# opteroncx/MoePhoto

Hardware: AMD Instinct MI355X
Metric: megapixels/sec (input), 1080p 4x SR (Net4x a4), 256-px tiles with overlap (higher is better)
Workload: dtype fp16; 1 GPU; BASELINE configs[1]: 1 frame(s) 1920x1080 RGB -> 7680x4320, model a4 (Net4x, synthetic weights in zoo format), crop 256 pad 5 align 8 -> 40 tiles/frame, fp16 I/O, fp16 MFMA operands + fp32 accumulate; tiles_per_frame=40, parallelism=single GPU, precision=mixed, exact_blocks=1, input=natural-image-like synthetic frame (tests/golden_defs.natural_image)

## Files before the change

### moephoto_amd/build.py

```python
import hashlib
import os
import subprocess
import sys

HERE = os.path.dirname(os.path.abspath(__file__))
CSRC = os.path.join(HERE, 'csrc')
SOURCES = ['conv_mfma.hip', 'conv3x3_sp.hip', 'conv3x3_rw.hip', 'conv3x3_ps4.hip', 'conv3x3_ps9.hip', 'arsb32c.hip', 'conv64_x3.hip', 'conv64_q8.hip', 'conv64_sq.hip', 'arsb_sq.hip', 'conv64_s.hip', 'conv1x1.hip', 'conv1x1_f2.hip', 'misc_kernels.hip', 'blend.hip', 'sym.hip',
           'errors.cpp', 'options.cpp', 'weights.cpp', 'forward.cpp', 'forward_arsb.cpp', 'forward_sedn.cpp', 'forward_lite.cpp', 'calibrate.cpp', 'plan_run.cpp', 'planner.cpp']
HEADERS = ['common.h', 'engine.h', 'net.h', 'rowtile.h', os.path.join('..', '..', 'include', 'moephoto_amd.h')]
LIB = os.path.join(HERE, 'libmoephoto_amd.so')
ARCH = 'gfx950'
EXTRA_FLAGS = {'blend.hip': ['-ffp-contract=off'],
               'sym.hip': ['-ffp-contract=off'],
               'arsb32c.hip': ['-fno-slp-vectorize', '-fno-honor-nans', '-mllvm', '-amdgpu-mfma-vgpr-form=1'], 'conv64_x3.hip': ['-fno-slp-vectorize'], 'conv64_q8.hip': ['-fno-slp-vectorize', '-fno-honor-nans', '-mllvm', '-amdgpu-mfma-vgpr-form=1'], 'conv64_sq.hip': ['-fno-slp-vectorize', '-fno-honor-nans', '-mllvm', '-amdgpu-mfma-vgpr-form=1'], 'arsb_sq.hip': ['-fno-slp-vectorize', '-fno-honor-nans', '-mllvm', '-amdgpu-mfma-vgpr-form=1'], 'conv64_s.hip': ['-fno-slp-vectorize', '-fno-honor-nans', '-mllvm', '-amdgpu-mfma-vgpr-form=1'], 'conv1x1.hip': ['-fno-slp-vectorize', '-mllvm', '-amdgpu-mfma-vgpr-form=1'], 'conv1x1_f2.hip': ['-fno-slp-vectorize', '-mllvm', '-amdgpu-mfma-vgpr-form=1'], 'conv3x3_sp.hip': ['-fno-honor-nans'], 'conv3x3_rw.hip': ['-fno-honor-nans', '-fno-slp-vectorize'],
               'conv3x3_ps4.hip': ['-fno-honor-nans', '-fno-slp-vectorize', '-mllvm', '-amdgpu-mfma-vgpr-form=1'],
               'conv3x3_ps9.hip': ['-fno-honor-nans', '-fno-slp-vectorize', '-mllvm', '-amdgpu-mfma-vgpr-form=1']}


def hipcc():
    for c in (os.environ.get('HIPCC'), '/opt/rocm/bin/hipcc', 'hipcc'):
        if c and (os.path.isabs(c) and os.path.exists(c) or not os.path.isabs(c)):
            return c
    return 'hipcc'


def source_digest():
    import hashlib
    h = hashlib.sha256()
    for f in sorted(SOURCES + HEADERS[:-1]) + HEADERS[-1:]:
        h.update(f.encode())
        h.update(open(os.path.join(CSRC, f), 'rb').read())
    return h.hexdigest()


def _compile_cmd(src, extra=()):
    obj = os.path.join(HERE, '_obj', os.path.splitext(src)[0] + '.o')
    cmd = [hipcc(), '--offload-arch=' + ARCH, '-O3', '-std=c++17', '-fPIC', '-x', 'hip', '-c', os.path.join(CSRC, src), '-o', obj]
    cmd += ['-cuid=moe_' + os.path.splitext(src)[0]]
    cmd += EXTRA_FLAGS.get(src, []) + list(extra)
    rel = [c.replace(CSRC, '<csrc>').replace(HERE, '<pkg>') for c in cmd[1:]]
    return cmd, hashlib.sha256('\0'.join(rel).encode()).hexdigest()


def stale():
    if not os.path.exists(LIB):
        return True
    t = os.path.getmtime(LIB)
    for src in SOURCES:
        tag = os.path.join(HERE, '_obj', os.path.splitext(src)[0] + '.o.cmd')
        if not os.path.exists(tag) or open(tag).read().strip() != _compile_cmd(src)[1]:
            return True
    return os.environ.get('MOE_HIPCC_FLAGS') is not None or any(os.path.getmtime(os.path.join(CSRC, f)) > t for f in SOURCES + HEADERS)


def build_lib(force=False, verbose=False):
    if not force and not stale():
        return LIB
    objs = []
    os.makedirs(os.path.join(HERE, '_obj'), exist_ok=True)
    keep = {os.path.splitext(src)[0] + e for src in SOURCES for e in ('.o', '.o.cmd')}
    for old in os.listdir(os.path.join(HERE, '_obj')):
        if old not in keep:
# ... 55 lines not shown
```

### moephoto_amd/csrc/conv3x3_ps4.hip

```cpp
#include "common.h"
#include "rowtile.h"
#include "../../include/moephoto_amd.h"
#include <algorithm>
#include <type_traits>

#ifndef PS4_FILL
#define PS4_FILL 5
#endif
#ifndef PS4_ZSKIP
#define PS4_ZSKIP 1
#endif
#ifndef PS4_ABL
#define PS4_ABL 0
#endif

namespace {

constexpr int RB = 4;
constexpr int PW = kTileW + 2;
constexpr int ROWB = PW * 128;
constexpr int BLKB = RB * ROWB;
constexpr int NPIECE = BLKB / 1024;
constexpr int TREC = 36 * 128 + 64;
constexpr int TEXP = 36 * 128;
constexpr int TROWS = 16;
constexpr int OFF_T = 2 * BLKB;
constexpr int OFF_BIAS = OFF_T + TROWS * TREC;
constexpr int OFF_TW = OFF_BIAS + 1024;
constexpr int OFF_DUMP = OFF_TW + 8 * 1024;
constexpr int LDS_BYTES = OFF_DUMP + 1024;

typedef unsigned u4_t __attribute__((ext_vector_type(4)));
typedef unsigned u2_t __attribute__((ext_vector_type(2)));
typedef float float2_t __attribute__((ext_vector_type(2)));
typedef const __attribute__((address_space(3))) half8_t* lds_h8_t;

enum OpKind : int { OP_NONE = 0, OP_P, OP_WL, OP_TM, OP_TW, OP_BI, OP_DMA, OP_FA, OP_FR, OP_FS, OP_AR, OP_AS, OP_ST };
struct Op { int kind, a, b, c; };
struct OpList {
    int n = 0;
    Op op[64] = {};
    constexpr void push(int kind, int a = 0, int b = 0, int c = 0) { op[n] = Op{kind, a, b, c}; ++n; }
    constexpr void append(const OpList& o) { for (int i = 0; i < o.n; ++i) { op[n] = o.op[i]; ++n; } }
};
constexpr OpList row_ops(int epi)
{
    OpList r;
    if (epi == 0) {
        for (int s = 0; s < 4; ++s) {
            r.push(OP_P, s >> 1, 4 * (s & 1), 2); r.push(OP_P, s >> 1, 4 * (s & 1) + 2, 2);
            r.push(OP_ST, s >> 1, s & 1);
        }
        return r;
    }
    const bool split = epi == 2;
    int nl = 0;
    auto wl = [&](int frag) { r.push(OP_WL, frag, nl & 1); ++nl; };
    int nt = 0;
    wl(0);
    wl(split ? 4 : 1);
    for (int s = 0; s < 4; ++s) {
        if (split) for (int k = 0; k < 4; ++k) r.push(OP_P, s >> 1, 4 * (s & 1) + k, 1);
        else for (int k = 0; k < 4; k += 2) r.push(OP_P, s >> 1, 4 * (s & 1) + k, 2);
        r.push(OP_TM, nt & 1, 0, nt == 0); ++nt;
        if (split) {
            if (s < 3) wl(s + 1);
            r.push(OP_TM, nt & 1, 1, 0); ++nt;
            if (s < 3) wl(4 + s + 1);
        } else if (s + 2 < 4) wl(s + 2);
    }
    for (int k = 0; k < 5; ++k) r.push(OP_TW, k);
// ... 91 lines not shown
    };
    auto piece_off = [&](int ya, int xa, bool live) {
        const bool ok = ((unsigned)(ya + (int)d_r) < (unsigned)H) & ((unsigned)(xa + (int)d_cc) < (unsigned)W) & live;
        return ok ? d_off : kOOR;
    };

    unsigned fa[3];
#pragma unroll
    for (int dx = 0; dx < 3; ++dx) {
        const int cc = j + dx, z = (cc >> 1) & 7;
        fa[dx] = lds0 + (unsigned)(cc * 128 + ((z ^ hh) << 4));
        asm volatile("" : "+v"(fa[dx]));
    }
    unsigned wa[5];
#pragma unroll
    for (int k = 0; k < 5; ++k) {
        const int t = k < 4 ? 4 * hh + k : 8;
        const int dy = t / 3, dx = t - 3 * dy;
        int col = j;
        if (pj == 1 && dx == 0) col = j + 1;
        if (pj == 0 && dx == 2) col = j - 1;
        unsigned o = (unsigned)((w4 * 9 + t) * 128 + col * 4);
        if (col == kTileW) o = (unsigned)(TEXP + ((0 * 2 + pi) * 3 + dy) * 4);
        if (col < 0) o = (unsigned)(TEXP + ((1 * 2 + pi) * 3 + dy) * 4);
        if (k == 4 && hh == 1) o = (unsigned)(TEXP + 48 + w4 * 4);
        wa[k] = lds0 + (unsigned)OFF_T + o;
        asm volatile("" : "+v"(wa[k]));
    }
    const int f_i = (lane >> 4) & 1, f_xp = lane & 15;
    const int a_side = (lane >> 1) & 1, a_i = lane & 1;
    unsigned slope2;
    {
        const half2_t s2 = {(half_t)a.slope, (half_t)a.slope};
        slope2 = __builtin_bit_cast(unsigned, s2);
    }
    const float16_t zero16 = {0.f, 0.f, 0.f, 0.f, 0.f, 0.f, 0.f, 0.f, 0.f, 0.f, 0.f, 0.f, 0.f, 0.f, 0.f, 0.f};

    float16_t acc[4][2];
    half8_t fr[3];
    half8_t twr[2];
    unsigned hX[4], lX[4];
    float16_t Gt = zero16;

    asm volatile("s_waitcnt lgkmcnt(0)" ::: "memory");
    __builtin_amdgcn_s_barrier();

    while (item < item_end) {
        const int s0 = item % nyb;
        const int t_ = item / nyb;
        const int pxi = t_ % px, b = t_ / px;
        const int s1 = min(nyb, s0 + (item_end - item));
        item += s1 - s0;
        const int x0 = pxi * kTileW;
        const int nblk = s1 - s0 + 3;
        const int kfirst = (PS4_ZSKIP && s0 == 0) ? 1 : 0;
        const int kz = (PS4_ZSKIP && s1 == nyb) ? nblk - 2 : nblk - 1;
        const bool okx = x0 + j < W;
        const int ylo = RB * s0, yhi = RB * s1;

        asm volatile("s_waitcnt lgkmcnt(0)" ::: "memory");
        __builtin_amdgcn_s_barrier();
        asm volatile("" ::: "memory");
        {
            const int ya = RB * (s0 - 1 + kfirst), xa = x0 - 1;
            const unsigned org = (unsigned)((b * H + ya + RB) * W + xa + 1) * 128u;
#pragma unroll
            for (int m = 0; m < 5; ++m) {
                piece_addr(m);
                const bool mine = m < 4 || w4 == 0;
                char* dst = smem + (m < 4 ? (w4 + 4 * m) * 1024 : (mine ? 16 * 1024 : OFF_DUMP));
                __builtin_amdgcn_raw_ptr_buffer_load_lds(rin, (__attribute__((address_space(3))) void*)dst, 16, piece_off(ya, xa, mine), org, 0, 0);
#if PS4_ABL & 128
                if (m < 4) __builtin_amdgcn_raw_ptr_buffer_load_lds(rin, (__attribute__((address_space(3))) void*)(dst + BLKB), 16, piece_off(ya + 4 * RB, xa, mine), org + (unsigned)(4 * RB * W) * 128u, 0, 0);
#endif
            }
#pragma unroll
            for (int s = 0; s < 4; ++s)
#pragma unroll
                for (int cg = 0; cg < 2; ++cg) acc[s][cg] = *(const __attribute__((address_space(3))) float16_t*)(bias_ad + cg * 128);
            asm volatile("s_waitcnt vmcnt(0) lgkmcnt(0)" ::: "memory");
            __builtin_amdgcn_s_barrier();
            asm volatile("" ::: "memory");
            fr[0] = *(lds_h8_t)(fa[0]);
            fr[1] = *(lds_h8_t)(fa[0] ^ 32u);
        }

        auto block = [&](int k, auto BUF_, auto KIND_) __attribute__((always_inline)) {
            constexpr int BUF = decltype(BUF_)::value;
            constexpr bool LAST = decltype(KIND_)::value == 2;
            constexpr bool ZERO = decltype(KIND_)::value == 1;
            const int Rk = RB * (s0 - 1 + k);
            const bool live = k + 1 < kz;
            const int yan = Rk + RB, xan = x0 - 1;
            const unsigned orgn = (unsigned)__builtin_amdgcn_readfirstlane((int)((unsigned)((b * H + yan + RB) * W + xan + 1) * 128u));
            const int yf = Rk - 7 + w4;
            const bool f_ok = (yf >= ylo) & (yf < yhi);
            unsigned fb[3];
            float2_t fs[2] = {{0.f, 0.f}, {0.f, 0.f}};
            float2_t fv[2];
            float av[3];

            auto step = [&](auto E_) __attribute__((always_inline)) {
                constexpr int e = decltype(E_)::value;
                const int orow = Rk + e - 2;
                const unsigned trow = (unsigned)__builtin_amdgcn_readfirstlane((int)((unsigned)((orow + 64) & 15) * (unsigned)TREC));
                const bool rowok = (unsigned)orow < (unsigned)H;
                constexpr int SL = (e + 2) & 3;

                auto op_p = [&](auto CG_, auto K0_, auto N_) __attribute__((always_inline)) {
                    constexpr int cg = decltype(CG_)::value, k0 = decltype(K0_)::value, n = decltype(N_)::value;
#pragma unroll
                    for (int k = k0; k < k0 + n; ++k) {
                        const float s0v = acc[SL][cg][2 * k], s1v = acc[SL][cg][2 * k + 1];
                        unsigned hv, lv = 0;
                        if (SPLIT) {
                            const float t0 = __builtin_fmaxf(s0v, s0v * a.slope), t1 = __builtin_fmaxf(s1v, s1v * a.slope);
                            split2(t0, t1, -2048.f, hv, lv);
                        } else {
                            const half2_t pr = {(half_t)s0v, (half_t)s1v};
                            const half2_t t = pr * __builtin_bit_cast(half2_t, slope2);
                            hv = __builtin_bit_cast(unsigned, __builtin_elementwise_max(pr, t));
                        }
                        hX[k & 3] = hv; lX[k & 3] = lv;
                    }
                };
                auto op_st = [&](auto CG_, auto G_) __attribute__((always_inline)) {
                    constexpr int cg = decltype(CG_)::value, gq = decltype(G_)::value;
                    const bool rok = (orow >= ylo) & (orow < yhi);
                    const unsigned vo = okx ? (unsigned)(2 * j) * 128u + (unsigned)hh * 16u : kOOR;
                    const unsigned so = rok ? ((unsigned)((b * 2 * H + 2 * orow + pi) * 2 * W + 2 * x0 + pj) * 128u + (unsigned)(64 * cg + 32 * gq)) : kOOR;
                    const u4_t d = {hX[0], hX[1], hX[2], hX[3]};
                    __builtin_amdgcn_raw_buffer_store_b128(d, rpl, vo, so, 0);
                };
                auto op_wl = [&](auto F_, auto S_) __attribute__((always_inline)) {
                    constexpr int fg = decltype(F_)::value, st = decltype(S_)::value;
                    twr[st] = *(lds_h8_t)(tw_ad + (unsigned)(fg * 1024));
                };
                auto op_tm = [&](auto S_, auto LO_, auto FIRST_) __attribute__((always_inline)) {
                    constexpr int st = decltype(S_)::value, lo = decltype(LO_)::value, first = decltype(FIRST_)::value;
                    const half8_t bv = lo ? __builtin_bit_cast(half8_t, u4_t{lX[0], lX[1], lX[2], lX[3]}) : __builtin_bit_cast(half8_t, u4_t{hX[0], hX[1], hX[2], hX[3]});
                    Gt = __builtin_amdgcn_mfma_f32_32x32x16_f16(twr[st], bv, first ? zero16 : Gt, 0, 0, 0);
                };
                auto op_tw = [&](auto K_) __attribute__((always_inline)) {
                    constexpr int k = decltype(K_)::value;
                    float t = __builtin_fmaf(Gt[8 + k], 0.00048828125f, Gt[k]);
                    const bool ok = MASK ? (rowok & okx) : rowok;
                    t = ok ? t : 0.f;
                    const unsigned ad = wa[k] + trow;
                    asm volatile("ds_write_b32 %0, %1" ::"v"(ad), "v"(t) : "memory");
                };
                auto op_bi = [&](auto CG_) __attribute__((always_inline)) {
                    constexpr int cg = decltype(CG_)::value;
#pragma unroll
                    for (int q = 0; q < 4; ++q) {
                        const float4_t t = *(const __attribute__((address_space(3))) float4_t*)(bias_ad + (unsigned)(cg * 128 + q * 16));
                        acc[SL][cg][4 * q] = t[0]; acc[SL][cg][4 * q + 1] = t[1]; acc[SL][cg][4 * q + 2] = t[2]; acc[SL][cg][4 * q + 3] = t[3];
// ... 12 lines not shown
#pragma unroll
                    for (int dy = 0; dy < 3; ++dy) {
                        const int isrc = f_i == 0 ? (dy == 1 ? 0 : 1) : (dy == 1 ? 1 : 0);
                        const int dd = f_i == 0 ? (dy == 0 ? -1 : 0) : (dy == 2 ? 1 : 0);
                        fb[dy] = lds0 + (unsigned)OFF_T + (unsigned)((yf + dd + 64) & 15) * (unsigned)TREC + (unsigned)((2 * isrc * 9 + dy * 3) * 128 + f_xp * 8);
                    }
                };
                auto op_fr = [&](auto DY_, auto DX_) __attribute__((always_inline)) {
                    constexpr int dy = decltype(DY_)::value, dx = decltype(DX_)::value;
                    constexpr int j0 = dx == 1 ? 0 : 1, j1 = dx == 1 ? 1 : 0;
                    if constexpr (dx > 0 || dy > 0) { fs[0] = fs[0] + fv[0]; fs[1] = fs[1] + fv[1]; }
                    fv[0] = *(const __attribute__((address_space(3))) float2_t*)(fb[dy] + (unsigned)((j0 * 9 + dx) * 128));
                    fv[1] = *(const __attribute__((address_space(3))) float2_t*)(fb[dy] + (unsigned)((j1 * 9 + dx) * 128));
                };
                auto op_fs = [&]() __attribute__((always_inline)) {
                    fs[0] = fs[0] + fv[0]; fs[1] = fs[1] + fv[1];
                    const float4_t o4 = {fs[0][0], fs[1][0], fs[0][1], fs[1][1]};
                    const bool ok = f_ok & (lane < 32) & (x0 + 2 * f_xp < W);
                    const unsigned vo = ok ? (unsigned)(f_i * 2 * W + 4 * f_xp) * 4u : kOOR;
                    const unsigned so = (unsigned)(((b * 2 * H + 2 * yf) * 2 * W) + 2 * x0) * 4u;
                    __builtin_amdgcn_raw_buffer_store_b128(__builtin_bit_cast(u4_t, o4), rpl, vo, f_ok ? so : 0u, 0);
                };
                auto op_ar = [&]() __attribute__((always_inline)) {
#pragma unroll
                    for (int dy = 0; dy < 3; ++dy) {
                        const int isrc = a_i == 0 ? (dy == 1 ? 0 : 1) : (dy == 1 ? 1 : 0);
                        const int dd = a_i == 0 ? (dy == 0 ? -1 : 0) : (dy == 2 ? 1 : 0);
                        const unsigned ad = lds0 + (unsigned)OFF_T + (unsigned)((yf + dd + 64) & 15) * (unsigned)TREC + (unsigned)(TEXP + ((a_side * 2 + isrc) * 3 + dy) * 4);
                        av[dy] = *(const __attribute__((address_space(3))) float*)ad;
                    }
                };
                auto op_as = [&]() __attribute__((always_inline)) {
                    const float v = (av[0] + av[1]) + av[2];
                    const bool ok = f_ok & (lane >= 32) & (lane < 36);
                    const unsigned vo = ok ? (unsigned)(((a_side * a.B) * px) * 2 * H + a_i) * 4u : kOOR;
                    const unsigned so = (unsigned)((b * px + pxi) * 2 * H + 2 * yf) * 4u;
                    __builtin_amdgcn_raw_buffer_store_b32(__builtin_bit_cast(unsigned, v), rap, vo, f_ok ? so : 0u, 0);
                };

                if constexpr (LAST) {
                    if constexpr (e == 0 && !(PS4_ABL & 2)) {
                        op_fa();
                        op_fr(std::integral_constant<int, 0>{}, std::integral_constant<int, 0>{}); op_fr(std::integral_constant<int, 0>{}, std::integral_constant<int, 1>{}); op_fr(std::integral_constant<int, 0>{}, std::integral_constant<int, 2>{});
                        op_fr(std::integral_constant<int, 1>{}, std::integral_constant<int, 0>{}); op_fr(std::integral_constant<int, 1>{}, std::integral_constant<int, 1>{}); op_fr(std::integral_constant<int, 1>{}, std::integral_constant<int, 2>{});
                        op_fr(std::integral_constant<int, 2>{}, std::integral_constant<int, 0>{}); op_fr(std::integral_constant<int, 2>{}, std::integral_constant<int, 1>{}); op_fr(std::integral_constant<int, 2>{}, std::integral_constant<int, 2>{});
                        op_fs();
                        op_ar(); op_as();
                    }
                    return;
                }
                auto chunk = [&](auto F_) __attribute__((always_inline)) {
                    constexpr int f = decltype(F_)::value;
                    constexpr int dx = f >> 2, ks = f & 3;
                    if (e == 3 && f == 10 && !(PS4_ABL & 16)) {
                        asm volatile("s_waitcnt vmcnt(0) lgkmcnt(0)" ::: "memory");
                        __builtin_amdgcn_s_barrier();
                        asm volatile("" ::: "memory");
                    }
                    constexpr OpList LM = row_ops(EPI);
                    constexpr OpList LX = extra_ops(e, TAIL);
                    auto half = [&](auto HC_) __attribute__((always_inline)) {
                        constexpr int hc = decltype(HC_)::value;
                        if constexpr (!ZERO) {
#pragma unroll
                            for (int u = 3 * hc; u < 3 * hc + 3; ++u) {
                                const int dy = u >> 1, cg = u & 1;
                                const int sl = (e + 1 - dy + 4) & 3;
                                acc[sl][cg] = __builtin_amdgcn_mfma_f32_32x32x16_f16(wf[cg][(dy * 3 + dx) * 4 + ks], fr[f % 3], acc[sl][cg], 0, 0, 0);
                            }
                        }
                        if constexpr (hc == 0 && !ZERO) {
                            constexpr int f2 = (f + 2) % 12;
                            constexpr int rowsel = f + 2 < 12 ? BUF * RB + e : (e < 3 ? BUF * RB + e + 1 : (BUF ^ 1) * RB);
                            if (!(PS4_ABL & 8)) fr[(f + 2) % 3] = *(lds_h8_t)((fa[f2 >> 2] ^ (unsigned)((f2 & 3) * 32)) + (unsigned)(rowsel * ROWB));
                        }
                        constexpr int h = 2 * f + hc;
                        constexpr int MH = TAIL ? 20 : 10;
                        constexpr int m_lo = h < MH ? h * LM.n / MH : LM.n, m_hi = h < MH ? (h + 1) * LM.n / MH : LM.n;
                        constexpr int x_lo = TAIL ? h * LX.n / 24 : (h < 12 ? 0 : (h - 12) * LX.n / 12), x_hi = TAIL ? (h + 1) * LX.n / 24 : (h < 12 ? 0 : (h - 11) * LX.n / 12);
                        auto runm = [&](auto I_) __attribute__((always_inline)) {
                            constexpr int I = decltype(I_)::value;
                            if constexpr (I >= m_lo && I < m_hi && !(PS4_ABL & 1)) {
                                constexpr Op o = LM.op[I];
                                if constexpr (o.kind == OP_P) op_p(std::integral_constant<int, o.a>{}, std::integral_constant<int, o.b>{}, std::integral_constant<int, o.c>{});
                                if constexpr (o.kind == OP_WL) op_wl(std::integral_constant<int, o.a>{}, std::integral_constant<int, o.b>{});
                                if constexpr (o.kind == OP_TM && !(PS4_ABL & 32)) op_tm(std::integral_constant<int, o.a>{}, std::integral_constant<int, o.b>{}, std::integral_constant<int, o.c>{});
                                if constexpr (o.kind == OP_TW) op_tw(std::integral_constant<int, o.a>{});
                                if constexpr (o.kind == OP_ST) op_st(std::integral_constant<int, o.a>{}, std::integral_constant<int, o.b>{});
                            }
                        };
                        auto runx = [&](auto I_) __attribute__((always_inline)) {
                            constexpr int I = decltype(I_)::value;
                            if constexpr (I >= x_lo && I < x_hi) {
                                constexpr Op o = LX.op[I];
                                if constexpr (o.kind != OP_DMA && (PS4_ABL & 2)) return;
                                if constexpr (o.kind == OP_DMA && (PS4_ABL & 64)) return;
                                if constexpr (o.kind == OP_DMA) op_dma(std::integral_constant<int, o.a>{}, std::integral_constant<int, o.b>{});
                                if constexpr (o.kind == OP_FA) op_fa();
                                if constexpr (o.kind == OP_FR) op_fr(std::integral_constant<int, o.a>{}, std::integral_constant<int, o.b>{});
                                if constexpr (o.kind == OP_FS) op_fs();
                                if constexpr (o.kind == OP_AR) op_ar();
                                if constexpr (o.kind == OP_AS) op_as();
                            }
                        };
#define PS4_M(I) runm(std::integral_constant<int, I>{});
                        PS4_M(0) PS4_M(1) PS4_M(2) PS4_M(3) PS4_M(4) PS4_M(5) PS4_M(6) PS4_M(7) PS4_M(8) PS4_M(9) PS4_M(10) PS4_M(11) PS4_M(12) PS4_M(13) PS4_M(14) PS4_M(15)
                        PS4_M(16) PS4_M(17) PS4_M(18) PS4_M(19) PS4_M(20) PS4_M(21) PS4_M(22) PS4_M(23) PS4_M(24) PS4_M(25) PS4_M(26) PS4_M(27) PS4_M(28) PS4_M(29) PS4_M(30) PS4_M(31)
                        PS4_M(32) PS4_M(33) PS4_M(34) PS4_M(35) PS4_M(36) PS4_M(37) PS4_M(38) PS4_M(39) PS4_M(40) PS4_M(41) PS4_M(42) PS4_M(43) PS4_M(44) PS4_M(45) PS4_M(46) PS4_M(47)
#undef PS4_M
#define PS4_X(I) runx(std::integral_constant<int, I>{});
                        PS4_X(0) PS4_X(1) PS4_X(2) PS4_X(3) PS4_X(4) PS4_X(5) PS4_X(6) PS4_X(7) PS4_X(8) PS4_X(9) PS4_X(10) PS4_X(11) PS4_X(12) PS4_X(13) PS4_X(14) PS4_X(15)
#undef PS4_X
                        if (f == 10 && hc == 1 && !(PS4_ABL & 4)) op_bi(std::integral_constant<int, 0>{});
                        if (f == 11 && hc == 1 && !(PS4_ABL & 4)) op_bi(std::integral_constant<int, 1>{});
                    };
                    half(std::integral_constant<int, 0>{});
                    half(std::integral_constant<int, 1>{});
#ifndef PS4_NOPIN
#pragma unroll
                    for (int hc = 0; hc < (ZERO ? 0 : 2); ++hc) {
                        const int h = 2 * f + hc;
                        const int MH = TAIL ? 20 : 10;
                        const int m_lo = h < MH ? h * LM.n / MH : LM.n, m_hi = h < MH ? (h + 1) * LM.n / MH : LM.n;
                        const int ntm = (PS4_ABL & 33) ? 0 : count_kind(LM, m_lo, m_hi, OP_TM);
#pragma unroll
                        for (int i_ = 0; i_ < 3; ++i_) {
                            __builtin_amdgcn_sched_group_barrier(0x008, 1, 0);
                            if (i_ == 0 && hc == 0) __builtin_amdgcn_sched_group_barrier(0x100, 1, 0);
                            __builtin_amdgcn_sched_group_barrier(0x006, PS4_FILL, 0);
                        }
#pragma unroll
                        for (int i_ = 0; i_ < 2; ++i_)
                            if (TAIL && i_ < ntm) { __builtin_amdgcn_sched_group_barrier(0x008, 1, 0); __builtin_amdgcn_sched_group_barrier(0x006, PS4_FILL, 0); }
                    }
#endif
                    __builtin_amdgcn_sched_barrier(0);
                };
#if PS4_ABL
                if constexpr (!LAST) asm volatile("" ::"v"(acc[SL][0]), "v"(acc[SL][1]), "v"(Gt));
#endif
#define PS4_CHUNK(F) chunk(std::integral_constant<int, F>{});
                PS4_CHUNK(0) PS4_CHUNK(1) PS4_CHUNK(2) PS4_CHUNK(3) PS4_CHUNK(4) PS4_CHUNK(5) PS4_CHUNK(6) PS4_CHUNK(7) PS4_CHUNK(8) PS4_CHUNK(9) PS4_CHUNK(10) PS4_CHUNK(11)
#undef PS4_CHUNK
            };
            step(std::integral_constant<int, 0>{});
            step(std::integral_constant<int, 1>{});
            step(std::integral_constant<int, 2>{});
            step(std::integral_constant<int, 3>{});
        };

        typedef std::integral_constant<int, 0> Run;
        typedef std::integral_constant<int, 1> Zero;
        typedef std::integral_constant<int, 2> Last;
        int k = kfirst;
        for (; k + 1 < kz; k += 2) {
            block(k, std::integral_constant<int, 0>{}, Run{});
            block(k + 1, std::integral_constant<int, 1>{}, Run{});
        }
        if (k < kz) { block(k, std::integral_constant<int, 0>{}, Run{}); ++k; }
        if (k < nblk - 1) { block(k, std::integral_constant<int, 0>{}, Zero{}); ++k; }
        if (TAIL) block(k, std::integral_constant<int, 0>{}, Last{});
    }
#endif
}

template <bool VEC>
__global__ __launch_bounds__(256) void tailadd_kernel(TailAddArgs a)
{
    const int nq = a.W >> 3;
    const long long idx = (long long)blockIdx.x * 256 + threadIdx.x;
    if (idx >= (long long)a.B * a.H * nq) return;
    const int xq = (int)(idx % nq);
    const int Y = (int)((idx / nq) % a.H), b = (int)(idx / ((long long)nq * a.H));
    const int X0 = xq * 8;
    const long long po = ((long long)b * a.H + Y) * a.W + X0;
    float v[8];
    {
        const float4 r0 = *(const float4*)(a.p0 + po), r1 = *(const float4*)(a.p0 + po + 4);
        v[0] = r0.x; v[1] = r0.y; v[2] = r0.z; v[3] = r0.w; v[4] = r1.x; v[5] = r1.y; v[6] = r1.z; v[7] = r1.w;
        if (a.p1) {
            const float4 u0 = *(const float4*)(a.p1 + po), u1 = *(const float4*)(a.p1 + po + 4);
            v[0] += u0.x; v[1] += u0.y; v[2] += u0.z; v[3] += u0.w; v[4] += u1.x; v[5] += u1.y; v[6] += u1.z; v[7] += u1.w;
        }
    }
    const int c = X0 >> 6, in = X0 & 63;
    const long long as = (long long)a.B * a.px * a.H;
    if (in == 0 && c >= 1) {
        const long long o = ((long long)b * a.px + (c - 1)) * a.H + Y;
        float t = a.a0[o];
        if (a.a1) t += a.a1[o];
        v[0] += t;
    }
    if (in == 56 && c + 1 < a.px) {
        const long long o = as + ((long long)b * a.px + (c + 1)) * a.H + Y;
        float t = a.a0[o];
        if (a.a1) t += a.a1[o];
        v[7] += t;
    }
    const long long yo = (a.y_off ? a.y_off[b] : (long long)b * a.H * a.W) + (long long)Y * a.W + X0;
    if (a.y_dtype == MOE_F16) {
        if (VEC) {
            half8_t h;
#pragma unroll
            for (int k = 0; k < 8; ++k) h[k] = (half_t)v[k];
            *(half8_t*)((half_t*)a.y + yo) = h;
        } else {
#pragma unroll
            for (int k = 0; k < 8; ++k) ((half_t*)a.y)[yo + k] = (half_t)v[k];
        }
    } else {
        float* yp = (float*)a.y + yo;
        if (VEC) {
            *(float4*)yp = make_float4(v[0], v[1], v[2], v[3]);
// ... 70 lines not shown
```

### moephoto_amd/csrc/forward.cpp

```cpp
#include "net.h"

using namespace moe;

namespace moe {

const char* kernel_name(ConvKernel k)
{
    static const char* const names[] = {"no kernel", "conv_direct", "conv1x1", "conv_mfma", "conv3x3_sp", "conv3x3_rw", "conv3x3_ps4 (store form)", "conv3x3_sp (hi + lo residual)",
                                        "conv_mfma (three products)", "conv64_x3", "conv64_q8", "conv64_sq", "conv3x3_sp (three launches)", "conv_mfma (fp32 side buffer)"};
    return names[(int)k];
}

static bool fast_layer(const moe_net& n, const ConvLayer& L) { return L.taps == 9 && L.nseg == 1 && !L.per_plane && n.opt.conv_impl == 2; }

ConvForm Fwd::form(const ConvLayer& L, int H, int W) const
{
    ConvForm c;
    c.B = B; c.H = H; c.W = W; c.in_cs = 64 * L.nseg; c.out_cs = L.r > 1 ? 64 : 64 * L.nchunks; c.r = L.r; c.nchunks = L.nchunks;
    c.py = (H + kTileH - 1) / kTileH;
    const long long items = (long long)B * ((W + kTileW - 1) / kTileW) * c.py;
    const int per_xcd = groups / 8;
    int G = per_xcd >= L.nchunks ? 8 * (per_xcd / L.nchunks) : groups / L.nchunks;
    if (G < 1) G = 1;
    if (G > items) G = (int)items;
    c.G = G;
    c.slope = L.slope; c.scale = L.scale; c.dbg = n.opt.dbg;
    return c;
}

ConvRoute Fwd::route(const std::string& key, const Act& in, const Act& out, const Act* res, int H, int W, const ConvExtra& e) const
{
    ConvRoute r;
    auto take = [&r](ConvKernel k) { r.kernel = k; return r; };
    auto refuse = [&r]() { r.kernel = ConvKernel::none; r.done.ok = false; return r; };
    const ConvLayer& L = n.convs[n.conv_index.at(key)];
    const bool x3 = this->x3 || e.exact;
    const bool res_lo = res && res->has_lo;
    const bool any8 = in.lo8 || out.lo8 || (res && res->lo8);
    if (any8 && !(x3 && use_q8() && q8_capable(L) && !direct)) return refuse();
    if (e.fuse_tail1) r.done.tail1_parts = 2;
    ConvForm& c = r.form;
    c = form(L, H, W);
    if (direct) return take(ConvKernel::direct);
    const int px = (W + kTileW - 1) / kTileW;
    c.res = res != nullptr; c.tail1 = e.fuse_tail1;
    c.tail = e.fuse_tail; c.tail_form = e.fuse_tail ? tail_form : 0; c.tail_split = (e.fuse_tail && mixed && tail_split_for(key)) ? 1 : 0;
    if (e.pool && !x3 && L.r == 1 && L.nchunks == 1 && !res && pooled_groups_ok((long long)c.py, (long long)B * c.py, groups)) {
        c.pool = true; c.pool_slabs = e.pool_slabs;
        c.G = pooled_groups((long long)c.py, (long long)B * c.py, groups);
    }
    const bool fast = fast_layer(n, L);
    if (e.fuse_tail && !(fast && !x3)) return refuse();
    if (n.opt.conv1x1 && L.taps == 1 && L.nseg == 1 && !L.per_plane && !res && L.scale == 1.f && !e.fuse_tail && n.opt.conv_impl == 2 && (!x3 || (in.has_lo && L.has_x3)) &&
        conv1x1_applicable(Conv1x1Form{B, H, W, L.r, L.nchunks, c.out_cs, L.slope, x3, e.fuse_tail1, x3 && out.has_lo}, groups)) {
        if (e.fuse_tail1) r.done.tail1_parts = 1;
        return take(ConvKernel::conv1x1);
    }
    const bool traced = !x3 && (c.dbg & 64) && fast && key == n.opt.trace_key;
    if (!x3 && !traced && res_lo && out.has_lo) {
        c.acc_mode = 3; c.side16 = true; c.out_lo = true;
        r.done.ok = fast && conv3x3_sp_applicable(c);
        return take(ConvKernel::sp_res_lo);
    }
    if (!x3) {
        if (c.tail && c.tail_form == 1) { r.done.ok = conv3x3_rw_applicable(c); return take(ConvKernel::rw); }
        if (fast && n.opt.up_impl == 1 && !c.tail && !c.pool && c.r == 2 && c.nchunks == 4 && c.in_cs == 64 && !c.res && c.scale == 1.f && !c.dbg && L.has_bias &&
            (long long)B * px * (H / 4) >= 32ll * groups && ps4_store_applicable(B, H, W, L.slope))
            return take(ConvKernel::ps4_store);
        if (fast && n.opt.sp_impl && !c.tail && conv3x3_rw_applicable(c)) { r.done.pooled = c.pool; return take(ConvKernel::rw); }
        if (fast && conv3x3_sp_applicable(c)) return take(ConvKernel::sp);
        if (c.tail) return refuse();
        return take(ConvKernel::mfma);
    }
    if (L.has_x3 && !fast) return take(ConvKernel::mfma_x3);
    if (n.opt.x3_fuse && fast && L.w_arsb_lo && in.has_lo && out.has_lo && (!res || res_lo) && !e.fuse_tail && !L.has_bias) {
        ConvX3Form q;
        q.B = B; q.H = H; q.W = W; q.slope = L.slope; q.res = res != nullptr; q.res_lo = res_lo;
        const long long P = (long long)px * c.py;
        if (e.pool && !res && (L.slope == 1.f || e.pool_act) && pooled_groups_ok(P, (long long)B * P, groups)) { q.pool = true; q.pool_slabs = e.pool_slabs; }
        if (e.gate && res && !use_q8()) q.gate = true;
        r.x3 = q;
        if (use_q8() && L.wq_hi8 && !q.pool && (!res || res->lo8 == in.lo8)) {
            r.x3.in8 = in.lo8; r.x3.out8 = out.lo8;
            if (n.opt.q8_impl == 1 && conv64_sq_applicable(r.x3, groups)) return take(ConvKernel::sq);
            if (conv64_q8_applicable(r.x3)) return take(ConvKernel::q8);
            r.x3 = q;
        }
        if (any8) return refuse();
        if (conv64_x3_applicable(q, groups)) { r.done.pooled = q.pool; r.done.gated = q.gate; return take(ConvKernel::x3); }
    }
    if (fast && L.nchunks <= 16) {
        ConvForm q1 = c; q1.res = res_lo; q1.slope = 1.f; q1.scale = 1.f; q1.tail = false;
        ConvForm q2 = q1; q2.res = true;
        ConvForm q3 = c; q3.acc_mode = 3; q3.side16 = true; q3.out_lo = out.has_lo;
        if (conv3x3_sp_applicable(q1) && conv3x3_sp_applicable(q2) && conv3x3_sp_applicable(q3)) return take(ConvKernel::sp_three);
    }
    if (!acc32_elems) return refuse();
    return take(ConvKernel::acc32);
}

int Fwd::launch(const ConvRoute& r, const std::string& key, const Act& in, const Act& out, const Act* res, const ConvExtra& e)
{
    const ConvLayer& L = n.convs[n.conv_index.at(key)];
    const ConvForm& c = r.form;
    const int H = c.H, W = c.W;
    if (r.kernel == ConvKernel::direct) {
        DirectConvArgs d{};
        d.in = in.hi; d.out = out.hi; d.res = res ? res->hi : nullptr;
        d.w = blob<float>(L.w_plain);
        d.bias = L.has_bias ? blob<float>(L.bias_plain) : nullptr;
        d.w_batch_stride = 0;
        d.B = B; d.H = H; d.W = W; d.in_cs = c.in_cs; d.out_cs = c.out_cs; d.cin = L.cin; d.cout = L.cout; d.k = L.k; d.r = L.r;
        d.slope = L.slope; d.scale = L.scale;
        if (L.per_plane) { d.w = (const float*)e.plane_w; d.w_batch_stride = (long long)L.cout * L.cin; }
        launch_conv_direct(d, s);
        return MOE_OK;
    }
    ConvArgs a{};
    a.in = in.hi; a.out = out.hi; a.res = res ? res->hi : nullptr;
    a.wpk = L.per_plane ? e.plane_w : blob<half_t>(L.w_hi);
    a.bias = L.has_bias ? blob<float>(L.bias) : small<float>("zero_bias");
    a.zero = small<half_t>("zero");
    a.bias_img = blob<float>(L.bias_img);
    a.trash = small<half_t>("trash");
    a.w_batch_stride = L.per_plane ? (long long)L.nchunks * L.nfrag() * 512 : 0;
    a.B = B; a.H = H; a.W = W; a.in_cs = c.in_cs; a.out_cs = c.out_cs; a.r = c.r; a.nchunks = c.nchunks;
    a.px = (W + kTileW - 1) / kTileW; a.py = c.py; a.G = c.G;
    a.slope = c.slope; a.scale = c.scale; a.dbg = c.dbg;
    a.tail_w = e.tail_w; a.tplanes = e.tplanes; a.tail_form = c.tail_form; a.tail_split = c.tail_split;
    a.tail1_w = e.tail1_w; a.tail1_out = e.tail1_out;
    if (c.pool) { a.pool = e.pool_out; a.pool_slabs = c.pool_slabs; }
    const bool x3 = this->x3 || e.exact;
    const bool timed = r.kernel != ConvKernel::mfma_x3 && r.kernel != ConvKernel::sp_three && r.kernel != ConvKernel::acc32;
    const int rec = timed ? prof_begin(key, (x3 ? 3 : 1) * 2.0 * (double)B * H * W * L.cout * L.cin * L.taps) : -1;
    bool ok = true;
    auto single = [&](const ConvArgs& ca) {
        if (r.kernel == ConvKernel::rw) return launch_conv3x3_rw(ca, s);
        if (r.kernel == ConvKernel::sp) return launch_conv3x3_sp(ca, s);
        if (r.kernel == ConvKernel::ps4_store) {
            Ps4Args q{};
            q.in = ca.in; q.wpk = ca.wpk; q.bias = ca.bias; q.out = ca.out; q.slope = ca.slope; q.B = ca.B; q.H = ca.H; q.W = ca.W;
            return launch_conv3x3_ps4(q, groups, s);
        }
        launch_conv_mfma(ca, L.taps, L.nseg, s);
        return true;
    };
    switch (r.kernel) {
    case ConvKernel::conv1x1: {
        Conv1x1Args q{};
        q.in_hi = in.hi; q.in_lo = x3 ? in.lo : nullptr; q.out_hi = out.hi; q.out_lo = x3 ? out.lo : nullptr;
        q.w_hi = blob<half_t>(L.w_hi); q.w_lo = x3 ? blob<half_t>(L.w_lo) : nullptr; q.bias = a.bias;
        q.tail_w = e.tail1_w; q.tail_out = e.tail1_out; q.slope = L.slope;
        q.B = B; q.H = H; q.W = W; q.r = L.r; q.nchunks = L.nchunks; q.out_cs = c.out_cs;
        q.nks = (L.cin <= 48 && n.opt.k48) ? 3 : 4;
        ok = launch_conv1x1(q, groups, s);
        break;
    }
    case ConvKernel::mfma: case ConvKernel::sp: case ConvKernel::rw: case ConvKernel::ps4_store: {
        unsigned long long* tr = nullptr;
        const size_t nb = 8 * 32 * 4 * 16 * 8;
        if (!x3 && (c.dbg & 64) && fast_layer(n, L) && key == n.opt.trace_key && hipMalloc((void**)&tr, nb) == hipSuccess) {
            (void)hipMemsetAsync(tr, 0, nb, s);
            ConvArgs t = a; t.acc32 = (float*)tr;
            ok = single(t);
            std::vector<unsigned long long> host(nb / 8);
            (void)hipStreamSynchronize(s);
            (void)hipMemcpy(host.data(), tr, nb, hipMemcpyDeviceToHost);
            if (FILE* f = fopen("/tmp/moe_trace.bin", "wb")) { fwrite(host.data(), 1, nb, f); fclose(f); }
            (void)hipFree(tr);
        } else
            ok = single(a);
        break;
    }
    case ConvKernel::sp_res_lo: {
        ConvArgs q = a; q.acc_mode = 3; q.side16 = res->lo; q.out_lo = out.lo; q.res_lo = nullptr;
        ok = launch_conv3x3_sp(q, s);
        break;
    }
    case ConvKernel::mfma_x3: {
        ConvArgs f4 = a; f4.wpk = blob<half_t>(L.w_x3); f4.acc_mode = 4; f4.in_lo = in.lo; f4.out_lo = out.lo; f4.res_lo = res ? res->lo : nullptr;
        launch_conv_mfma(f4, 1, 3, s);
        break;
    }
    case ConvKernel::x3: case ConvKernel::q8: case ConvKernel::sq: {
        ConvX3Args q{};
        q.in_hi = in.hi; q.in_lo = in.lo; q.out_hi = out.hi; q.out_lo = out.lo;
        q.res_hi = res ? res->hi : nullptr; q.res_lo = res ? res->lo : nullptr;
        q.w_hi = blob<half_t>(L.w_arsb); q.w_lo = blob<half_t>(L.w_arsb_lo); q.zero = small<half_t>("zero");
        q.slope = L.slope; q.B = B; q.H = H; q.W = W;
        if (r.x3.pool) { q.pool = e.pool_out; q.pool_slabs = e.pool_slabs; }
        if (r.x3.gate) q.gate = e.gate_in;
        if (r.kernel == ConvKernel::x3) { ok = launch_conv64_x3(q, groups, s); break; }
        q.wq_hi16 = blob<half_t>(L.w_hi); q.wq_hi8 = blob<unsigned char>(L.wq_hi8); q.wq_lo8 = blob<unsigned char>(L.wq_lo8);
        q.in8 = r.x3.in8; q.out8 = r.x3.out8;
        ok = r.kernel == ConvKernel::sq ? launch_conv64_sq(q, groups, s) : launch_conv64_q8(q, groups, s);
        break;
    }
    case ConvKernel::sp_three: {
        ConvArgs q1 = a; q1.wpk = blob<half_t>(L.w_lo); q1.out = side16; q1.res = (res && res->has_lo) ? res->lo : nullptr; q1.bias = small<float>("zero_bias");
        q1.bias_img = small<float>("zero_bias_img"); q1.slope = 1.f; q1.scale = 1.f; q1.acc_mode = 0; q1.tail_w = nullptr; q1.tplanes = nullptr;
        ConvArgs q2 = q1; q2.in = in.lo; q2.wpk = blob<half_t>(L.w_hi); q2.res = side16;
        ConvArgs q3 = a; q3.acc_mode = 3; q3.side16 = side16; q3.out_lo = out.lo; q3.res_lo = nullptr;
        ok = launch_conv3x3_sp(q1, s) && launch_conv3x3_sp(q2, s) && launch_conv3x3_sp(q3, s);
        break;
    }
    case ConvKernel::acc32: {
        a.acc32 = acc32;
        ConvArgs p1 = a; p1.wpk = L.per_plane ? e.plane_w_lo : blob<half_t>(L.w_lo); p1.acc_mode = 1; p1.res = nullptr; p1.bias = nullptr;
        launch_conv_mfma(p1, L.taps, L.nseg, s);
        ConvArgs p2 = a; p2.in = in.lo; p2.acc_mode = 2; p2.res = nullptr; p2.bias = nullptr;
        launch_conv_mfma(p2, L.taps, L.nseg, s);
        ConvArgs p3 = a; p3.acc_mode = 3; p3.out_lo = out.lo; p3.res_lo = res ? res->lo : nullptr;
        launch_conv_mfma(p3, L.taps, L.nseg, s);
        break;
    }
    default: ok = false;
    }
    prof_end(rec);
    if (!ok) return fail(MOE_EINVAL, "internal error: layer %s (%d planes of %dx%d) was routed to %s, and that launcher refused it", key.c_str(), B, H, W, kernel_name(r.kernel));
    return MOE_OK;
}

ConvDone Fwd::conv(const std::string& key, const Act& in, const Act& out, const Act* res, int H, int W, const ConvExtra& e)
{
// ... 415 lines not shown
```

Baseline: 87.58 MP/s.

## Trim MFMAs in ps4 strip edge blocks to only rows the strip needs

Adds special Above and Below edge-block kinds to the pixel-shuffle conv3x3 kernel. These run only the MFMAs and epilogue ops that feed rows the strip owns, instead of computing full halo blocks. The halo rows above are prefetched alongside the first block, and compile-time tables with static_assert checks verify that every wanted output row is still covered. The planner also drops the minimum-work threshold for choosing ps4_store. A repeats() loop is added around single-kernel launches, which looks like profiling support.

Result: no change. 87.63 MP/s (median of 5 runs) (+0.1%).

```diff
diff --git a/moephoto_amd/build.py b/moephoto_amd/build.py
--- a/moephoto_amd/build.py
+++ b/moephoto_amd/build.py
@@ -7,7 +7,7 @@
 CSRC = os.path.join(HERE, 'csrc')
 SOURCES = ['conv_mfma.hip', 'conv3x3_sp.hip', 'conv3x3_rw.hip', 'conv3x3_ps4.hip', 'conv3x3_ps9.hip', 'arsb32c.hip', 'conv64_x3.hip', 'conv64_q8.hip', 'conv64_sq.hip', 'arsb_sq.hip', 'conv64_s.hip', 'conv1x1.hip', 'conv1x1_f2.hip', 'misc_kernels.hip', 'blend.hip', 'sym.hip',
            'errors.cpp', 'options.cpp', 'weights.cpp', 'forward.cpp', 'forward_arsb.cpp', 'forward_sedn.cpp', 'forward_lite.cpp', 'calibrate.cpp', 'plan_run.cpp', 'planner.cpp']
-HEADERS = ['common.h', 'engine.h', 'net.h', 'rowtile.h', os.path.join('..', '..', 'include', 'moephoto_amd.h')]
+HEADERS = ['common.h', 'engine.h', 'net.h', 'rowtile.h', 'ps4_edges.h', os.path.join('..', '..', 'include', 'moephoto_amd.h')]
 LIB = os.path.join(HERE, 'libmoephoto_amd.so')
 ARCH = 'gfx950'
 EXTRA_FLAGS = {'blend.hip': ['-ffp-contract=off'],
diff --git a/moephoto_amd/csrc/conv3x3_ps4.hip b/moephoto_amd/csrc/conv3x3_ps4.hip
--- a/moephoto_amd/csrc/conv3x3_ps4.hip
+++ b/moephoto_amd/csrc/conv3x3_ps4.hip
@@ -1,5 +1,6 @@
 #include "common.h"
 #include "rowtile.h"
+#include "ps4_edges.h"
 #include "../../include/moephoto_amd.h"
 #include <algorithm>
 #include <type_traits>
@@ -16,7 +17,7 @@
 
 namespace {
 
-constexpr int RB = 4;
+constexpr int RB = kPs4RB;
 constexpr int PW = kTileW + 2;
 constexpr int ROWB = PW * 128;
 constexpr int BLKB = RB * ROWB;
@@ -214,9 +215,10 @@
         const int s1 = min(nyb, s0 + (item_end - item));
         item += s1 - s0;
         const int x0 = pxi * kTileW;
-        const int nblk = s1 - s0 + 3;
-        const int kfirst = (PS4_ZSKIP && s0 == 0) ? 1 : 0;
-        const int kz = (PS4_ZSKIP && s1 == nyb) ? nblk - 2 : nblk - 1;
+        const int kb = s1 - s0 + 1;
+        const bool has_above = !(PS4_ZSKIP && s0 == 0);
+        const bool zero_below = PS4_ZSKIP && s1 == nyb;
+        const int kin = zero_below ? kb : kb + 1;
         const bool okx = x0 + j < W;
         const int ylo = RB * s0, yhi = RB * s1;
 
@@ -224,7 +226,7 @@
         __builtin_amdgcn_s_barrier();
         asm volatile("" ::: "memory");
         {
-            const int ya = RB * (s0 - 1 + kfirst), xa = x0 - 1;
+            const int ya = RB * s0, xa = x0 - 1;
             const unsigned org = (unsigned)((b * H + ya + RB) * W + xa + 1) * 128u;
 #pragma unroll
             for (int m = 0; m < 5; ++m) {
@@ -232,6 +234,8 @@
                 const bool mine = m < 4 || w4 == 0;
                 char* dst = smem + (m < 4 ? (w4 + 4 * m) * 1024 : (mine ? 16 * 1024 : OFF_DUMP));
                 __builtin_amdgcn_raw_ptr_buffer_load_lds(rin, (__attribute__((address_space(3))) void*)dst, 16, piece_off(ya, xa, mine), org, 0, 0);
+                char* dsta = smem + (m < 4 ? BLKB + (w4 + 4 * m) * 1024 : (mine ? BLKB + 16 * 1024 : OFF_DUMP));
+                __builtin_amdgcn_raw_ptr_buffer_load_lds(rin, (__attribute__((address_space(3))) void*)dsta, 16, piece_off(ya - RB, xa, mine & has_above), org - (unsigned)(RB * W) * 128u, 0, 0);
 #if PS4_ABL & 128
                 if (m < 4) __builtin_amdgcn_raw_ptr_buffer_load_lds(rin, (__attribute__((address_space(3))) void*)(dst + BLKB), 16, piece_off(ya + 4 * RB, xa, mine), org + (unsigned)(4 * RB * W) * 128u, 0, 0);
 #endif
@@ -243,16 +247,21 @@
             asm volatile("s_waitcnt vmcnt(0) lgkmcnt(0)" ::: "memory");
             __builtin_amdgcn_s_barrier();
             asm volatile("" ::: "memory");
-            fr[0] = *(lds_h8_t)(fa[0]);
-            fr[1] = *(lds_h8_t)(fa[0] ^ 32u);
+            const unsigned first_row = has_above ? (unsigned)(BLKB + ps4_above_first(TAIL) * ROWB) : 0u;
+            fr[0] = *(lds_h8_t)(fa[0] + first_row);
+            fr[1] = *(lds_h8_t)((fa[0] ^ 32u) + first_row);
         }
 
         auto block = [&](int k, auto BUF_, auto KIND_) __attribute__((always_inline)) {
             constexpr int BUF = decltype(BUF_)::value;
-            constexpr bool LAST = decltype(KIND_)::value == 2;
-            constexpr bool ZERO = decltype(KIND_)::value == 1;
+            constexpr int KIND = decltype(KIND_)::value;
+            constexpr bool LAST = KIND == PS4_LAST;
+            constexpr bool ZERO = KIND == PS4_ZERO;
+            constexpr bool ABOVE = KIND == PS4_ABOVE, BELOW = KIND == PS4_BELOW;
+            constexpr bool RELOAD = KIND == PS4_RUN || ZERO;
+            const unsigned ring_off = BELOW ? (unsigned)(ps4_ring_half(k) * BLKB) : 0u;
             const int Rk = RB * (s0 - 1 + k);
-            const bool live = k + 1 < kz;
+            const bool live = k + 1 < kin;
             const int yan = Rk + RB, xan = x0 - 1;
             const unsigned orgn = (unsigned)__builtin_amdgcn_readfirstlane((int)((unsigned)((b * H + yan + RB) * W + xan + 1) * 128u));
             const int yf = Rk - 7 + w4;
@@ -264,6 +273,10 @@
 
             auto step = [&](auto E_) __attribute__((always_inline)) {
                 constexpr int e = decltype(E_)::value;
+                constexpr int NR = ps4_mfma_rows(TAIL, KIND, e);
+                constexpr bool EP = ps4_epilogue_runs(TAIL, KIND, e);
+                constexpr bool BAR = e == 3 && !BELOW;
+                if constexpr (!LAST && NR == 0 && !EP && !BAR) return;
                 const int orow = Rk + e - 2;
                 const unsigned trow = (unsigned)__builtin_amdgcn_readfirstlane((int)((unsigned)((orow + 64) & 15) * (unsigned)TREC));
                 const bool rowok = (unsigned)orow < (unsigned)H;
@@ -382,7 +395,8 @@
                 auto chunk = [&](auto F_) __attribute__((always_inline)) {
                     constexpr int f = decltype(F_)::value;
                     constexpr int dx = f >> 2, ks = f & 3;
-                    if (e == 3 && f == 10 && !(PS4_ABL & 16)) {
+                    constexpr bool NEXT = f + 2 < 12 || (e < 3 ? ps4_mfma_rows(TAIL, KIND, e < 3 ? e + 1 : 0) > 0 : !BELOW);
+                    if (BAR && f == 10 && !(PS4_ABL & 16)) {
                         asm volatile("s_waitcnt vmcnt(0) lgkmcnt(0)" ::: "memory");
                         __builtin_amdgcn_s_barrier();
                         asm volatile("" ::: "memory");
@@ -391,18 +405,18 @@
                     constexpr OpList LX = extra_ops(e, TAIL);
                     auto half = [&](auto HC_) __attribute__((always_inline)) {
                         constexpr int hc = decltype(HC_)::value;
-                        if constexpr (!ZERO) {
+                        if constexpr (NR > 0) {
 #pragma unroll
                             for (int u = 3 * hc; u < 3 * hc + 3; ++u) {
                                 const int dy = u >> 1, cg = u & 1;
                                 const int sl = (e + 1 - dy + 4) & 3;
-                                acc[sl][cg] = __builtin_amdgcn_mfma_f32_32x32x16_f16(wf[cg][(dy * 3 + dx) * 4 + ks], fr[f % 3], acc[sl][cg], 0, 0, 0);
+                                if (ps4_mfma_runs(TAIL, KIND, e, dy)) acc[sl][cg] = __builtin_amdgcn_mfma_f32_32x32x16_f16(wf[cg][(dy * 3 + dx) * 4 + ks], fr[f % 3], acc[sl][cg], 0, 0, 0);
                             }
                         }
-                        if constexpr (hc == 0 && !ZERO) {
+                        if constexpr (hc == 0 && NR > 0 && NEXT) {
                             constexpr int f2 = (f + 2) % 12;
                             constexpr int rowsel = f + 2 < 12 ? BUF * RB + e : (e < 3 ? BUF * RB + e + 1 : (BUF ^ 1) * RB);
-                            if (!(PS4_ABL & 8)) fr[(f + 2) % 3] = *(lds_h8_t)((fa[f2 >> 2] ^ (unsigned)((f2 & 3) * 32)) + (unsigned)(rowsel * ROWB));
+                            if (!(PS4_ABL & 8)) fr[(f + 2) % 3] = *(lds_h8_t)((fa[f2 >> 2] ^ (unsigned)((f2 & 3) * 32)) + ring_off + (unsigned)(rowsel * ROWB));
                         }
                         constexpr int h = 2 * f + hc;
                         constexpr int MH = TAIL ? 20 : 10;
@@ -410,7 +424,7 @@
                         constexpr int x_lo = TAIL ? h * LX.n / 24 : (h < 12 ? 0 : (h - 12) * LX.n / 12), x_hi = TAIL ? (h + 1) * LX.n / 24 : (h < 12 ? 0 : (h - 11) * LX.n / 12);
                         auto runm = [&](auto I_) __attribute__((always_inline)) {
                             constexpr int I = decltype(I_)::value;
-                            if constexpr (I >= m_lo && I < m_hi && !(PS4_ABL & 1)) {
+                            if constexpr (EP && I >= m_lo && I < m_hi && !(PS4_ABL & 1)) {
                                 constexpr Op o = LM.op[I];
                                 if constexpr (o.kind == OP_P) op_p(std::integral_constant<int, o.a>{}, std::integral_constant<int, o.b>{}, std::integral_constant<int, o.c>{});
                                 if constexpr (o.kind == OP_WL) op_wl(std::integral_constant<int, o.a>{}, std::integral_constant<int, o.b>{});
@@ -421,8 +435,9 @@
                         };
                         auto runx = [&](auto I_) __attribute__((always_inline)) {
                             constexpr int I = decltype(I_)::value;
-                            if constexpr (I >= x_lo && I < x_hi) {
+                            if constexpr (!ABOVE && I >= x_lo && I < x_hi) {
                                 constexpr Op o = LX.op[I];
+                                if constexpr (o.kind == OP_DMA && BELOW) return;
                                 if constexpr (o.kind != OP_DMA && (PS4_ABL & 2)) return;
                                 if constexpr (o.kind == OP_DMA && (PS4_ABL & 64)) return;
                                 if constexpr (o.kind == OP_DMA) op_dma(std::integral_constant<int, o.a>{}, std::integral_constant<int, o.b>{});
@@ -441,22 +456,25 @@
 #define PS4_X(I) runx(std::integral_constant<int, I>{});
                         PS4_X(0) PS4_X(1) PS4_X(2) PS4_X(3) PS4_X(4) PS4_X(5) PS4_X(6) PS4_X(7) PS4_X(8) PS4_X(9) PS4_X(10) PS4_X(11) PS4_X(12) PS4_X(13) PS4_X(14) PS4_X(15)
 #undef PS4_X
-                        if (f == 10 && hc == 1 && !(PS4_ABL & 4)) op_bi(std::integral_constant<int, 0>{});
-                        if (f == 11 && hc == 1 && !(PS4_ABL & 4)) op_bi(std::integral_constant<int, 1>{});
+                        if (RELOAD && f == 10 && hc == 1 && !(PS4_ABL & 4)) op_bi(std::integral_constant<int, 0>{});
+                        if (RELOAD && f == 11 && hc == 1 && !(PS4_ABL & 4)) op_bi(std::integral_constant<int, 1>{});
                     };
                     half(std::integral_constant<int, 0>{});
                     half(std::integral_constant<int, 1>{});
 #ifndef PS4_NOPIN
-#pragma unroll
-                    for (int hc = 0; hc < (ZERO ? 0 : 2); ++hc) {
+                    bool first = NEXT;
+#pragma unroll
+                    for (int hc = 0; hc < (NR == 0 ? 0 : 2); ++hc) {
                         const int h = 2 * f + hc;
                         const int MH = TAIL ? 20 : 10;
                         const int m_lo = h < MH ? h * LM.n / MH : LM.n, m_hi = h < MH ? (h + 1) * LM.n / MH : LM.n;
-                        const int ntm = (PS4_ABL & 33) ? 0 : count_kind(LM, m_lo, m_hi, OP_TM);
-#pragma unroll
-                        for (int i_ = 0; i_ < 3; ++i_) {
+                        const int ntm = ((PS4_ABL & 33) || !EP) ? 0 : count_kind(LM, m_lo, m_hi, OP_TM);
+                        const int nm = hc == 0 ? 2 * (int)ps4_mfma_runs(TAIL, KIND, e, 0) + (int)ps4_mfma_runs(TAIL, KIND, e, 1) : (int)ps4_mfma_runs(TAIL, KIND, e, 1) + 2 * (int)ps4_mfma_runs(TAIL, KIND, e, 2);
+#pragma unroll
+                        for (int i_ = 0; i_ < nm; ++i_) {
                             __builtin_amdgcn_sched_group_barrier(0x008, 1, 0);
-                            if (i_ == 0 && hc == 0) __builtin_amdgcn_sched_group_barrier(0x100, 1, 0);
+                            if (first) __builtin_amdgcn_sched_group_barrier(0x100, 1, 0);
+                            first = false;
                             __builtin_amdgcn_sched_group_barrier(0x006, PS4_FILL, 0);
                         }
 #pragma unroll
@@ -477,18 +495,28 @@
             step(std::integral_constant<int, 1>{});
             step(std::integral_constant<int, 2>{});
             step(std::integral_constant<int, 3>{});
+            if constexpr (BELOW && TAIL && !(PS4_ABL & 16)) {
+                asm volatile("s_waitcnt vmcnt(0) lgkmcnt(0)" ::: "memory");
+                __builtin_amdgcn_s_barrier();
+                asm volatile("" ::: "memory");
+            }
         };
 
-        typedef std::integral_constant<int, 0> Run;
-        typedef std::integral_constant<int, 1> Zero;
-        typedef std::integral_constant<int, 2> Last;
-        int k = kfirst;
-        for (; k + 1 < kz; k += 2) {
+        typedef std::integral_constant<int, PS4_RUN> Run;
+        typedef std::integral_constant<int, PS4_ZERO> Zero;
+        typedef std::integral_constant<int, PS4_LAST> Last;
+        typedef std::integral_constant<int, PS4_ABOVE> Above;
+        typedef std::integral_constant<int, PS4_BELOW> Below;
+        if (has_above) block(0, std::integral_constant<int, 1>{}, Above{});
+        int k = 1;
+        for (; k + 1 < kb; k += 2) {
             block(k, std::integral_constant<int, 0>{}, Run{});
             block(k + 1, std::integral_constant<int, 1>{}, Run{});
         }
-        if (k < kz) { block(k, std::integral_constant<int, 0>{}, Run{}); ++k; }
-        if (k < nblk - 1) { block(k, std::integral_constant<int, 0>{}, Zero{}); ++k; }
+        if (k < kb) { block(k, std::integral_constant<int, 0>{}, Run{}); ++k; }
+        if (zero_below) block(k, std::integral_constant<int, 0>{}, Zero{});
+        else block(k, std::integral_constant<int, 0>{}, Below{});
+        ++k;
         if (TAIL) block(k, std::integral_constant<int, 0>{}, Last{});
     }
 #endif
diff --git a/moephoto_amd/csrc/forward.cpp b/moephoto_amd/csrc/forward.cpp
--- a/moephoto_amd/csrc/forward.cpp
+++ b/moephoto_amd/csrc/forward.cpp
@@ -65,7 +65,7 @@
     if (!x3) {
         if (c.tail && c.tail_form == 1) { r.done.ok = conv3x3_rw_applicable(c); return take(ConvKernel::rw); }
         if (fast && n.opt.up_impl == 1 && !c.tail && !c.pool && c.r == 2 && c.nchunks == 4 && c.in_cs == 64 && !c.res && c.scale == 1.f && !c.dbg && L.has_bias &&
-            (long long)B * px * (H / 4) >= 32ll * groups && ps4_store_applicable(B, H, W, L.slope))
+            ps4_store_applicable(B, H, W, L.slope))
             return take(ConvKernel::ps4_store);
         if (fast && n.opt.sp_impl && !c.tail && conv3x3_rw_applicable(c)) { r.done.pooled = c.pool; return take(ConvKernel::rw); }
         if (fast && conv3x3_sp_applicable(c)) return take(ConvKernel::sp);
@@ -169,7 +169,7 @@
             if (FILE* f = fopen("/tmp/moe_trace.bin", "wb")) { fwrite(host.data(), 1, nb, f); fclose(f); }
             (void)hipFree(tr);
         } else
-            ok = single(a);
+            for (int rep = repeats(key); rep > 0; --rep) ok = single(a);
         break;
     }
     case ConvKernel::sp_res_lo: {
diff --git a/moephoto_amd/csrc/ps4_edges.h b/moephoto_amd/csrc/ps4_edges.h
--- /dev/null
+++ b/moephoto_amd/csrc/ps4_edges.h
@@ -0,0 +1,101 @@
+#pragma once
+
+enum Ps4Kind : int { PS4_RUN = 0, PS4_ZERO = 1, PS4_LAST = 2, PS4_ABOVE = 3, PS4_BELOW = 4 };
+
+constexpr int kPs4RB = 4;
+
+constexpr bool ps4_mfma_runs(bool tail, int kind, int e, int dy)
+{
+    if (kind == PS4_RUN) return true;
+    if (kind == PS4_ABOVE) return (e - kPs4RB + 1 - dy) >= (tail ? -1 : 0);
+    if (kind == PS4_BELOW) return (e + 1 - dy) <= (tail ? 0 : -1);
+    return false;
+}
+constexpr bool ps4_epilogue_runs(bool tail, int kind, int e)
+{
+    if (kind == PS4_RUN || kind == PS4_ZERO) return true;
+    if (kind == PS4_BELOW) return (e - 2) <= (tail ? 0 : -1);
+    return false;
+}
+constexpr int ps4_mfma_rows(bool tail, int kind, int e) { return (int)ps4_mfma_runs(tail, kind, e, 0) + (int)ps4_mfma_runs(tail, kind, e, 1) + (int)ps4_mfma_runs(tail, kind, e, 2); }
+constexpr int ps4_above_first(bool tail) { return ps4_mfma_rows(tail, PS4_ABOVE, 0) ? 0 : ps4_mfma_rows(tail, PS4_ABOVE, 1) ? 1 : ps4_mfma_rows(tail, PS4_ABOVE, 2) ? 2 : 3; }
+
+constexpr int ps4_kind(bool tail, bool zskip, int k, int s0, int s1, int nyb)
+{
+    const int n = s1 - s0;
+    if (k == 0) return (zskip && s0 == 0) ? -1 : PS4_ABOVE;
+    if (k <= n) return PS4_RUN;
+    if (k == n + 1) return (zskip && s1 == nyb) ? PS4_ZERO : PS4_BELOW;
+    return (k == n + 2 && tail) ? PS4_LAST : -1;
+}
+constexpr int ps4_ring_half(int k) { return (k + 1) & 1; }
+
+constexpr bool ps4_check_strip(bool tail, bool zskip, int s0, int s1, int nyb)
+{
+    const int H = kPs4RB * nyb, ylo = kPs4RB * s0, yhi = kPs4RB * s1;
+    const int want_lo = tail ? ylo - 1 : ylo, want_hi = tail ? yhi + 1 : yhi;
+    int got[3][64] = {}, last_in[64] = {}, epi[64] = {}, epi_at[64] = {};
+    const int CLEAN = -100, DIRTY = -99;
+    int owner[4] = {CLEAN, CLEAN, CLEAN, CLEAN};
+    for (int i = 0; i < 64; ++i) last_in[i] = -100;
+    const int OFF = 8;
+    for (int k = 0; k <= s1 - s0 + 2; ++k) {
+        const int kind = ps4_kind(tail, zskip, k, s0, s1, nyb);
+        if (kind < 0 || kind == PS4_LAST) continue;
+        const int Rk = kPs4RB * (s0 - 1 + k);
+        for (int e = 0; e < kPs4RB; ++e) {
+            const int r = Rk + e;
+            for (int dy = 0; dy < 3; ++dy) {
+                if (!ps4_mfma_runs(tail, kind, e, dy)) continue;
+                const int o = r + 1 - dy, sl = o & 3;
+                const bool wanted = o >= want_lo && o < want_hi;
+                if (kind != PS4_RUN && !wanted) return false;
+                if (owner[sl] >= want_lo && owner[sl] != o) return false;
+                if (!wanted) { owner[sl] = DIRTY; continue; }
+                if (owner[sl] == DIRTY) return false;
+                owner[sl] = o;
+                if (r <= last_in[o + OFF]) return false;
+                last_in[o + OFF] = r;
+                ++got[dy][o + OFF];
+            }
+            if (ps4_epilogue_runs(tail, kind, e)) {
+                const int o = r - 2, sl = o & 3;
+                if (o >= want_lo && o < want_hi) {
+                    ++epi[o + OFF];
+                    epi_at[o + OFF] = r;
+                    if (o >= 0 && o < H && owner[sl] != o) return false;
+                } else if (owner[sl] >= want_lo) return false;
+                owner[sl] = (kind == PS4_RUN || kind == PS4_ZERO) ? CLEAN : DIRTY;
+            }
+        }
+    }
+    for (int o = want_lo; o < want_hi; ++o) {
+        if (epi[o + OFF] != 1) return false;
+        if (o < 0 || o >= H) continue;
+        for (int dy = 0; dy < 3; ++dy) {
+            const int r = o - 1 + dy;
+            if (got[dy][o + OFF] != ((r >= 0 && r < H) || !zskip ? 1 : 0)) return false;
+        }
+        if (last_in[o + OFF] > epi_at[o + OFF]) return false;
+    }
+    return true;
+}
+constexpr bool ps4_check_all(bool tail, bool zskip)
+{
+    for (int nyb = 1; nyb <= 6; ++nyb)
+        for (int s0 = 0; s0 < nyb; ++s0)
+            for (int s1 = s0 + 1; s1 <= nyb; ++s1)
+                if (!ps4_check_strip(tail, zskip, s0, s1, nyb)) return false;
+    return true;
+}
+static_assert(ps4_check_all(false, true) && ps4_check_all(true, true), "conv3x3_ps4: the edge blocks' table does not cover the rows a strip wants");
+static_assert(ps4_check_all(false, false) && ps4_check_all(true, false), "conv3x3_ps4 (PS4_ZSKIP 0): the edge blocks' table does not cover the rows a strip wants");
+constexpr int ps4_edge_mfmas(bool tail, int kind)
+{
+    int n = 0;
+    for (int e = 0; e < kPs4RB; ++e) n += 24 * ps4_mfma_rows(tail, kind, e);
+    return n;
+}
+static_assert(ps4_edge_mfmas(false, PS4_ABOVE) == 24 && ps4_edge_mfmas(false, PS4_BELOW) == 24 && ps4_edge_mfmas(true, PS4_ABOVE) == 72 && ps4_edge_mfmas(true, PS4_BELOW) == 72 &&
+              ps4_edge_mfmas(true, PS4_RUN) == 288, "conv3x3_ps4: MFMAs of an edge block");
+static_assert(ps4_above_first(false) == 3 && ps4_above_first(true) == 2, "conv3x3_ps4: the Above block's first live input row");
```
